# AOADMM-DataFusionFramework/Matlab-Code

Measured on AMD Instinct MI355X. Metric: AO-ADMM outer iters/sec (+ mode-1 MTTKRP GFLOP/s), 2000^3 rank-20 CP, higher is better.
Workload: dtype f32

## Files before the change

### matlab-code_amd/csrc/contract.hip

```cpp
#include "contract.h"
#include "device_utils.h"
#include "small_dev.h"

#include <algorithm>
#include <cstdlib>

namespace aoadmm {

typedef float f32x4 __attribute__((ext_vector_type(4)));
typedef double f64x2 __attribute__((ext_vector_type(2)));
typedef double f64x4 __attribute__((ext_vector_type(4)));

static constexpr int kTileRows = 128;
static constexpr int kGroup = 8;

struct KArgs {
  const void* X;
  const void* frag;
  void* T;
  int64_t tiles_per_batch, ntiles, batch_stride, M, ld, C, Cg, trows;
  int groups_per_chunk, R;
  int flush_every;
};

// ... 677 lines not shown
  const int64_t ng = g1 > g0 ? g1 - g0 : 0;
  const _Float16* xp = a.X + (blk * a.Cg + g0) * kGroupHalves + (m0 + r16) * kGroup16 + 8 * q;
  const f16x8* fp = reinterpret_cast<const f16x8*>(reinterpret_cast<const char*>(a.frag) + kFragHeader16) + g0 * (NT * 128) + lane;

  f32x4 acc[NT][8];
#pragma unroll
  for (int nt = 0; nt < NT; ++nt)
#pragma unroll
    for (int t = 0; t < 8; ++t) acc[nt][t] = f32x4{0.f, 0.f, 0.f, 0.f};

  f16x8 x0[8], x1[8], x2[8];
  f16x8 f0[NT][2], f1[NT][2], f2[NT][2];
#define AO_LOAD1(XS, GI, TL) XS[TL] = __builtin_nontemporal_load(reinterpret_cast<const f16x8*>(xp + (GI) * kGroupHalves + (TL) * (16 * kGroup16)));
#define AO_LOADF(FS, GI)                                                                             \
  {                                                                                                  \
    _Pragma("unroll") for (int nt = 0; nt < NT; ++nt) {                                              \
      FS[nt][0] = fp[(GI) * (NT * 128) + nt * 128];                                                  \
      FS[nt][1] = fp[(GI) * (NT * 128) + nt * 128 + 64];                                             \
    }                                                                                                \
  }
#define AO_LOAD_STAGE(XS, FS, GI)                                                                    \
  { _Pragma("unroll") for (int tl_ = 0; tl_ < 8; ++tl_) AO_LOAD1(XS, GI, tl_) AO_LOADF(FS, GI) }
#define AO_FMA_T(XS, FS, TL)                                                                         \
  {                                                                                                  \
    _Pragma("unroll") for (int nt = 0; nt < NT; ++nt) {                                              \
      acc[nt][TL] = __builtin_amdgcn_mfma_f32_16x16x32_f16(XS[TL], FS[nt][0], acc[nt][TL], 0, 0, 0); \
      acc[nt][TL] = __builtin_amdgcn_mfma_f32_16x16x32_f16(XS[TL], FS[nt][1], acc[nt][TL], 0, 0, 0); \
    }                                                                                                \
  }
#define AO_COMPUTE_STAGE(XS, FS) { _Pragma("unroll") for (int tl_ = 0; tl_ < 8; ++tl_) AO_FMA_T(XS, FS, tl_) }
#define AO_MIX_STAGE(XC, FC, XL, FL, GI)                                                             \
  {                                                                                                  \
    _Pragma("unroll") for (int tl_ = 0; tl_ < 8; ++tl_) {                                            \
      AO_FMA_T(XC, FC, tl_) AO_LOAD1(XL, GI, tl_)                                                    \
      if (tl_ == 7) AO_LOADF(FL, GI)                                                                 \
      __builtin_amdgcn_sched_barrier(0);                                                             \
    }                                                                                                \
  }
  if (ng > 0) AO_LOAD_STAGE(x0, f0, 0)
  if (ng > 1) AO_LOAD_STAGE(x1, f1, 1)
  int64_t g = 0;
  for (; g + 5 <= ng; g += 3) {
    AO_MIX_STAGE(x0, f0, x2, f2, g + 2)
    AO_MIX_STAGE(x1, f1, x0, f0, g + 3)
    AO_MIX_STAGE(x2, f2, x1, f1, g + 4)
  }
  for (; g + 3 <= ng; g += 3) {
    if (g + 2 < ng) AO_LOAD_STAGE(x2, f2, g + 2)
    AO_COMPUTE_STAGE(x0, f0)
    if (g + 3 < ng) AO_LOAD_STAGE(x0, f0, g + 3)
    AO_COMPUTE_STAGE(x1, f1)
    if (g + 4 < ng) AO_LOAD_STAGE(x1, f1, g + 4)
    AO_COMPUTE_STAGE(x2, f2)
  }
  if (g < ng) AO_COMPUTE_STAGE(x0, f0)
  if (g + 1 < ng) AO_COMPUTE_STAGE(x1, f1)
#undef AO_LOAD1
#undef AO_LOADF
#undef AO_LOAD_STAGE
#undef AO_FMA_T
#undef AO_COMPUTE_STAGE
#undef AO_MIX_STAGE
  extern __shared__ __attribute__((aligned(16))) float t_lds[];
  float* tl = t_lds + (threadIdx.x >> 6) * (kTileRows * a.R);
  const float* tinv = reinterpret_cast<const float*>(reinterpret_cast<const char*>(a.frag) + 512);
#pragma unroll
  for (int nt = 0; nt < NT; ++nt) {
    const int r = 16 * nt + r16;
    if (r < a.R) {
      const float ti = tinv[r];
#pragma unroll
      for (int t = 0; t < 8; ++t)
#pragma unroll
        for (int i = 0; i < 4; ++i) tl[(16 * t + 4 * q + i) * a.R + r] = acc[nt][t][i] * ti * a.inv_s;
    }
  }
  {
    const int n16 = kTileRows * a.R / 4;
    f32x4* dst = reinterpret_cast<f32x4*>(a.T + ((int64_t)chunk * a.trows + blk * 512 + m0) * a.R);
    const f32x4* src = reinterpret_cast<const f32x4*>(tl);
    for (int c = lane; c < n16; c += 64) __builtin_nontemporal_store(src[c], dst + c);
  }
}

static int nt_of(int R, int prec) {
  const int w = prec == AOADMM_PREC_F32 ? 32 : 16;
  return (R + w - 1) / w;
}
static int tile_rows(int prec) { return prec == AOADMM_PREC_F64 ? kTileRows64 : kTileRows; }

size_t ContractPlan::frag_bytes(int prec) const {
  if (prec == AOADMM_PREC_F16)
    return (size_t)kFragHeader16 + (size_t)cdiv(C, kGroup16) * nt_of(R, prec) * 2048;
  const int64_t Cg = cdiv(C, kGroup);
  return (size_t)(nt_of(R, prec) * 1024 + 1152) * Cg + 8192;
}

ContractPlan make_plan(int64_t nbatch, int64_t batch_stride, int64_t M, int64_t ld, int64_t C, int R,
                       int prec) {
  ContractPlan p;
  const bool half = prec == AOADMM_PREC_F16;
  p.tprec = half ? AOADMM_PREC_F32 : prec;
  p.nbatch = nbatch; p.batch_stride = batch_stride; p.M = M; p.ld = ld; p.C = C; p.R = R;
  const int gcols = half ? kGroup16 : kGroup;
  const int64_t Cg = cdiv(C, gcols);
  const int64_t ntiles = nbatch * cdiv(M, tile_rows(prec));
  int64_t nchunk = 1;
  if (prec != AOADMM_PREC_F64) nchunk = cdiv(Cg, 2048 / gcols);
  if (ntiles < 2048) {
    int64_t want = cdiv(2048, ntiles);
    const int64_t gmin = 128 / gcols;
    int64_t maxc = Cg / gmin > 0 ? Cg / gmin : 1;
    if (want > maxc) want = maxc;
    if (want > nchunk) nchunk = want;
  }
  if (nchunk > 65535) nchunk = 65535;
  p.nchunk = (int)nchunk;
  return p;
}

ContractPlan make_lead_plan(int64_t M, int64_t ld, int64_t C, int R) {
  ContractPlan p;
  p.tprec = AOADMM_PREC_F32;
  p.nbatch = 1; p.batch_stride = 0; p.M = M; p.ld = ld; p.C = C; p.R = R;
  p.lead = true;
  const int64_t nch = cdiv(C, kLeadKC);
  p.nchunk = (int)cdiv(nch, 2048 / kLeadKC);
  return p;
}

static void launch_contract_lead(const void* X, const ContractPlan& pl, const double* F, int64_t ldF, void* frag_ws,
                                 void* T, hipStream_t s, hipEvent_t ev0, hipEvent_t ev1) {
  const int64_t Cg = cdiv(pl.C, kGroup);
  AO_REQUIRE(pl.ld % 4 == 0 && pl.ld >= 4, "f32 layout must be padded to 4");
  LArgs a;
  a.X = (const float*)X; a.frag = (const float*)frag_ws; a.T = (float*)T;
  a.M = pl.M; a.ld = pl.ld; a.C = pl.C; a.Cg = Cg; a.R = pl.R;
  a.chunks_per_slice = (int)cdiv(cdiv(pl.C, kLeadKC), pl.nchunk);
  const int64_t nblk = cdiv(pl.M, kLeadRows);
  AO_REQUIRE(nblk < (int64_t)2147483647, "tensor too large for one launch");
  dim3 grid((unsigned)nblk, (unsigned)pl.nchunk);
  const size_t sh = (size_t)2 * kLeadRows * kLeadStride * sizeof(float);
  const int nt16 = (pl.R + 15) / 16;
  const int64_t Cg16 = cdiv(pl.C, 16) + 1;
  const int64_t total = (int64_t)nt16 * Cg16 * 256;
  pack_frag_lead16_f32<<<(unsigned)cdiv(total, 256), 256, 0, s>>>(F, ldF, pl.C, pl.R, nt16, Cg16, (float*)frag_ws);
  AO_KERNEL_CHECK();
#define AO_SET(K) ensure_dynamic_lds(reinterpret_cast<const void*>(K), (int)sh);
  if (nt16 == 1) AO_SET(contract_lead16_f32<1>)
  else if (nt16 == 2) AO_SET(contract_lead16_f32<2>)
  else if (nt16 == 3) AO_SET(contract_lead16_f32<3>)
  else if (nt16 == 4) AO_SET(contract_lead16_f32<4>)
#undef AO_SET
  if (ev0) AO_HIP(hipEventRecord(ev0, s));
  if (nt16 == 1) contract_lead16_f32<1><<<grid, 256, sh, s>>>(a);
  else if (nt16 == 2) contract_lead16_f32<2><<<grid, 256, sh, s>>>(a);
  else if (nt16 == 3) contract_lead16_f32<3><<<grid, 256, sh, s>>>(a);
  else if (nt16 == 4) contract_lead16_f32<4><<<grid, 256, sh, s>>>(a);
  else throw Error(AOADMM_ERR_UNSUPPORTED, "rank > 64 not supported");
  if (ev1) AO_HIP(hipEventRecord(ev1, s));
  AO_KERNEL_CHECK();
}

static void launch_contract_half(const void* X, const ContractPlan& pl, const double* F, int64_t ldF, void* frag_ws,
                                 void* T, hipStream_t s, hipEvent_t ev0, hipEvent_t ev1) {
  AO_REQUIRE(pl.on_copy && !pl.lead && pl.M == 512 && pl.ld == 512 && pl.tprec == AOADMM_PREC_F32,
             "internal: a half operand is streamed from its pass copies only");
  const int64_t Cg = cdiv(pl.C, kGroup16);
  AO_REQUIRE(pl.batch_stride == 512 * kGroup16 * Cg && pl.nbatch > 0 && pl.C > 0, "internal: half pass copy and plan disagree");
  const int NT = nt_of(pl.R, AOADMM_PREC_F16);
  char* ws = reinterpret_cast<char*>(frag_ws);
  double* tsc = reinterpret_cast<double*>(ws);
  float* tinv = reinterpret_cast<float*>(ws + 512);
  frag16_scales_k<<<(unsigned)pl.R, 256, 0, s>>>(F, ldF, pl.C, tsc, tinv);
  AO_KERNEL_CHECK();
  pack_frag16_f16<<<(unsigned)cdiv(Cg * NT * 128, 256), 256, 0, s>>>(F, ldF, pl.C, pl.R, NT, Cg, tsc,
                                                                    reinterpret_cast<f16x8*>(ws + kFragHeader16));
  AO_KERNEL_CHECK();
  KArgs16 a;
  a.X = reinterpret_cast<const _Float16*>(X); a.frag = frag_ws; a.T = reinterpret_cast<float*>(T);
  a.ntiles = pl.nbatch * 4; a.Cg = Cg; a.trows = pl.trows();
  a.groups_per_chunk = (int)cdiv(Cg, pl.nchunk);
  a.R = pl.R;
  a.inv_s = (float)(1.0 / pl.xscale);
  AO_REQUIRE(pl.nbatch < (int64_t)2147483647, "tensor too large for one launch");
  const dim3 grid((unsigned)pl.nbatch, (unsigned)pl.nchunk);
  const size_t tsh = (size_t)4 * kTileRows * pl.R * sizeof(float);
#define AO_GO(K) { if (tsh > 65536) ensure_dynamic_lds(reinterpret_cast<const void*>(K), (int)tsh); if (ev0) AO_HIP(hipEventRecord(ev0, s)); K<<<grid, 256, tsh, s>>>(a); }
  if (NT == 1) AO_GO(contract16_f16<1>)
  else if (NT == 2) AO_GO(contract16_f16<2>)
  else if (NT == 3) AO_GO(contract16_f16<3>)
  else if (NT == 4) AO_GO(contract16_f16<4>)
  else throw Error(AOADMM_ERR_UNSUPPORTED, "rank > 64 not supported");
#undef AO_GO
  if (ev1) AO_HIP(hipEventRecord(ev1, s));
  AO_KERNEL_CHECK();
}

void launch_contract(const void* X, int prec, const ContractPlan& pl, const double* F, int64_t ldF,
                     void* frag_ws, void* T, hipStream_t s, hipEvent_t ev0, hipEvent_t ev1) {
  AO_REQUIRE(pl.R >= 1 && pl.R <= kMaxRank, "rank %d outside [1,%d]", pl.R, kMaxRank);
  if (prec == AOADMM_PREC_F16) {
    launch_contract_half(X, pl, F, ldF, frag_ws, T, s, ev0, ev1);
    return;
  }
  AO_REQUIRE(prec == AOADMM_PREC_F32 || prec == AOADMM_PREC_F64, "bad precision id %d", prec);
  AO_REQUIRE(pl.tprec == prec, "contraction plan and tensor precision disagree");
  if (pl.lead) {
    AO_REQUIRE(prec == AOADMM_PREC_F32, "leading-mode contraction exists for fp32 tensors only");
    launch_contract_lead(X, pl, F, ldF, frag_ws, T, s, ev0, ev1);
    return;
  }
  const int64_t Cg = cdiv(pl.C, kGroup);
  KArgs a;
  a.X = X; a.frag = frag_ws; a.T = T;
  a.tiles_per_batch = cdiv(pl.M, tile_rows(prec));
  a.ntiles = pl.nbatch * a.tiles_per_batch;
  a.batch_stride = pl.batch_stride; a.M = pl.M; a.ld = pl.ld; a.C = pl.C; a.Cg = Cg;
  a.trows = pl.trows();
  a.groups_per_chunk = (int)cdiv(Cg, pl.nchunk);
  a.R = pl.R;
  AO_REQUIRE(a.ntiles > 0 && pl.C > 0, "empty contraction");
  dim3 grid((unsigned)cdiv(a.ntiles, 4), (unsigned)pl.nchunk);
  AO_REQUIRE(cdiv(a.ntiles, 4) < (int64_t)2147483647, "tensor too large for one launch");
  if (prec == AOADMM_PREC_F32) {
    AO_REQUIRE(pl.ld % 4 == 0 && pl.M % 4 == 0 && pl.batch_stride % 4 == 0, "f32 layout must be padded to 4");
    const int rem = pl.R % 16;
    const bool ex = pl.R > 16 && rem >= 1 && rem <= 4;
    const int nt16 = ex ? pl.R / 16 : (pl.R + 15) / 16;
    const int64_t total = (int64_t)nt16 * Cg * 128 + (ex ? Cg * 32 : 0);
    pack_frag16_f32<<<(unsigned)cdiv(total, 256), 256, 0, s>>>(F, ldF, pl.C, pl.R, nt16, ex ? 1 : 0, Cg, (float*)frag_ws);
    AO_KERNEL_CHECK();
    size_t tsh = (size_t)4 * kTileRows * pl.R * sizeof(float);
    a.flush_every = kFlushEvery;
    if (nt16 == 1) tsh = (size_t)4 * 16384;
#define AO_GO(K) { if (tsh > 65536) ensure_dynamic_lds(reinterpret_cast<const void*>(K), (int)tsh); if (ev0) AO_HIP(hipEventRecord(ev0, s)); K<<<grid, 256, tsh, s>>>(a); }
    if (nt16 == 1 && !ex) AO_GO((contract16_f32<1, false, true>))
    else if (nt16 == 1) AO_GO((contract16_f32<1, true, true>))
    else if (nt16 == 2 && !ex) AO_GO((contract16_f32<2, false>))
    else if (nt16 == 2) AO_GO((contract16_f32<2, true>))
    else if (nt16 == 3 && !ex) AO_GO((contract16_f32<3, false>))
    else if (nt16 == 3) AO_GO((contract16_f32<3, true>))
    else if (nt16 == 4) AO_GO((contract16_f32<4, false>))
    else throw Error(AOADMM_ERR_UNSUPPORTED, "rank > 64 not supported");
#undef AO_GO
  } else {
    AO_REQUIRE(pl.ld % 2 == 0 && pl.M % 2 == 0 && pl.batch_stride % 2 == 0, "f64 layout must be padded to 2");
    const int rem = pl.R % 16;
    const bool ex = pl.R > 16 && rem >= 1 && rem <= 4;
    const int nt16 = ex ? pl.R / 16 : (pl.R + 15) / 16;
    const int64_t total = (int64_t)nt16 * Cg * 128 + (ex ? Cg * 32 : 0);
    pack_frag_f64<<<(unsigned)cdiv(total, 256), 256, 0, s>>>(F, ldF, pl.C, pl.R, nt16, ex ? 1 : 0, Cg, (double*)frag_ws);
    AO_KERNEL_CHECK();
    const size_t tsh = (size_t)4 * kTileRows64 * pl.R * sizeof(double);
#define AO_GO(K) { if (tsh > 65536) ensure_dynamic_lds(reinterpret_cast<const void*>(K), (int)tsh); if (ev0) AO_HIP(hipEventRecord(ev0, s)); K<<<grid, 256, tsh, s>>>(a); }
    if (nt16 == 1 && !ex) AO_GO((contract_f64<1, false>))
    else if (nt16 == 1) AO_GO((contract_f64<1, true>))
    else if (nt16 == 2 && !ex) AO_GO((contract_f64<2, false>))
    else if (nt16 == 2) AO_GO((contract_f64<2, true>))
    else if (nt16 == 3 && !ex) AO_GO((contract_f64<3, false>))
    else if (nt16 == 3) AO_GO((contract_f64<3, true>))
    else if (nt16 == 4) AO_GO((contract_f64<4, false>))
    else throw Error(AOADMM_ERR_UNSUPPORTED, "rank > 64 not supported");
#undef AO_GO
  }
  if (ev1) AO_HIP(hipEventRecord(ev1, s));
  AO_KERNEL_CHECK();
}

__global__ void factor_rowmajor_k(const double* __restrict__ F, int64_t ldF, int64_t rows, int R,
                                  double* __restrict__ Ft) {
  const int64_t idx = (int64_t)blockIdx.x * blockDim.x + threadIdx.x;
  if (idx >= rows * R) return;
  const int r = (int)(idx / rows);
  const int64_t a = idx - (int64_t)r * rows;
  Ft[a * R + r] = F[a + ldF * r];
}
static void factor_rowmajor(const double* F, int64_t ldF, int64_t rows, int R, double* Ft, hipStream_t s) {
  factor_rowmajor_k<<<(unsigned)cdiv(rows * R, 256), 256, 0, s>>>(F, ldF, rows, R, Ft);
  AO_KERNEL_CHECK();
}

template <typename TT, int VEC> struct TVec;
template <> struct TVec<float, 4> { typedef float type __attribute__((ext_vector_type(4))); };
template <> struct TVec<float, 1> { typedef float type; };
template <> struct TVec<double, 2> { typedef double type __attribute__((ext_vector_type(2))); };
template <> struct TVec<double, 1> { typedef double type; };
template <typename TT, int VEC>
__device__ __forceinline__ void fma_vec(double (&acc)[VEC], const TT* __restrict__ tp, const double* __restrict__ fp) {
  typedef typename TVec<TT, VEC>::type V;
  const V tv = __builtin_nontemporal_load(reinterpret_cast<const V*>(tp));
  if constexpr (VEC == 1) {
    acc[0] += (double)tv * fp[0];
  } else {
#pragma unroll
    for (int v = 0; v < VEC; ++v) acc[v] += (double)tv[v] * fp[v];
  }
}

template <typename TT, int VEC>
struct RVec {
  typename TVec<TT, VEC>::type t;
  double f[VEC];
  __device__ __forceinline__ void load(const TT* __restrict__ tp, const double* __restrict__ fp) {
    t = __builtin_nontemporal_load(reinterpret_cast<const typename TVec<TT, VEC>::type*>(tp));
#pragma unroll
    for (int v = 0; v < VEC; ++v) f[v] = fp[v];
  }
  __device__ __forceinline__ void fma(double (&acc)[VEC]) const {
    if constexpr (VEC == 1) {
      acc[0] += (double)t * f[0];
    } else {
#pragma unroll
      for (int v = 0; v < VEC; ++v) acc[v] += (double)t[v] * f[v];
    }
  }
};

template <typename TT, int VEC>
__global__ void reduce_inner_k(const TT* __restrict__ T, int nchunk, int64_t trows, int64_t A, int64_t Apad, int R,
                               const double* __restrict__ FaT, double scale, double* __restrict__ out,
                               int64_t ldOut, int rowmajor, int has_sys, SysBuild sys) {
  extern __shared__ double sh[];
  if (has_sys && blockIdx.x == 0) { sys_build_rider(sys); return; }
  const int64_t b = (int64_t)blockIdx.x - has_sys;
  const int t = threadIdx.x;
  const int64_t n = A * R, step = (int64_t)blockDim.x * VEC;
  double s0[VEC], s1[VEC], s2[VEC], s3[VEC];
#pragma unroll
  for (int v = 0; v < VEC; ++v) { s0[v] = 0; s1[v] = 0; s2[v] = 0; s3[v] = 0; }
  for (int ch = 0; ch < nchunk; ++ch) {
    const TT* Tb = T + ((int64_t)ch * trows + Apad * b) * R;
    int64_t e = (int64_t)t * VEC;
    for (; e + 3 * step < n; e += 4 * step) {
      RVec<TT, VEC> q0, q1, q2, q3;
      q0.load(Tb + e, FaT + e);
      q1.load(Tb + e + step, FaT + e + step);
      q2.load(Tb + e + 2 * step, FaT + e + 2 * step);
      q3.load(Tb + e + 3 * step, FaT + e + 3 * step);
      __builtin_amdgcn_sched_barrier(0);
      q0.fma(s0); q1.fma(s1); q2.fma(s2); q3.fma(s3);
    }
    for (; e < n; e += step) fma_vec<TT, VEC>(s0, Tb + e, FaT + e);
  }
#pragma unroll
  for (int v = 0; v < VEC; ++v) sh[t * VEC + v] = (s0[v] + s1[v]) + (s2[v] + s3[v]);
  __syncthreads();
  if (t < R) {
    const int nA = blockDim.x * VEC / R;
    double tot = 0.0;
    for (int i = 0; i < nA; ++i) tot += sh[i * R + t];
    if (rowmajor) out[b * R + t] = scale * tot;
    else out[b + ldOut * t] = scale * tot;
  }
}

template <typename TT, int VEC>
__global__ void reduce_inner2_k(const TT* __restrict__ T, int nchunk, int64_t trows, int64_t A, int64_t Apad, int64_t B,
                                int R, const double* __restrict__ FaT, double scale, double* __restrict__ out,
                                int64_t ldOut, int rowmajor, int has_sys, SysBuild sys) {
  extern __shared__ double sh[];
  if (has_sys && blockIdx.x == 0) { sys_build_rider(sys); return; }
  const int64_t b0 = 2 * ((int64_t)blockIdx.x - has_sys);
  const bool two = b0 + 1 < B;
  const int64_t b1 = two ? b0 + 1 : b0;
  const int t = threadIdx.x;
  const int64_t n = A * R, step = (int64_t)blockDim.x * VEC;
  double a0[VEC], a1[VEC], c0[VEC], c1[VEC];
#pragma unroll
  for (int v = 0; v < VEC; ++v) { a0[v] = 0; a1[v] = 0; c0[v] = 0; c1[v] = 0; }
  for (int ch = 0; ch < nchunk; ++ch) {
    const TT* Ta = T + ((int64_t)ch * trows + Apad * b0) * R;
    const TT* Tc = T + ((int64_t)ch * trows + Apad * b1) * R;
    int64_t e = (int64_t)t * VEC;
    for (; e + step < n; e += 2 * step) {
      RVec<TT, VEC> q0, q1, p0, p1;
      q0.load(Ta + e, FaT + e);
      q1.load(Ta + e + step, FaT + e + step);
      p0.t = __builtin_nontemporal_load(reinterpret_cast<const typename TVec<TT, VEC>::type*>(Tc + e));
      p1.t = __builtin_nontemporal_load(reinterpret_cast<const typename TVec<TT, VEC>::type*>(Tc + e + step));
      __builtin_amdgcn_sched_barrier(0);
#pragma unroll
      for (int v = 0; v < VEC; ++v) { p0.f[v] = q0.f[v]; p1.f[v] = q1.f[v]; }
      q0.fma(a0); q1.fma(a1); p0.fma(c0); p1.fma(c1);
    }
    for (; e < n; e += step) {
      RVec<TT, VEC> q0, p0;
      q0.load(Ta + e, FaT + e);
      p0.t = __builtin_nontemporal_load(reinterpret_cast<const typename TVec<TT, VEC>::type*>(Tc + e));
#pragma unroll
      for (int v = 0; v < VEC; ++v) p0.f[v] = q0.f[v];
      q0.fma(a0); p0.fma(c0);
    }
  }
  const int nt = blockDim.x * VEC;
#pragma unroll
  for (int v = 0; v < VEC; ++v) { sh[t * VEC + v] = a0[v] + a1[v]; sh[nt + t * VEC + v] = c0[v] + c1[v]; }
  __syncthreads();
  if (t < 2 * R) {
    const int which = t / R, r = t % R;
    if (which == 0 || two) {
      const int nA = nt / R;
      double tot = 0.0;
      for (int i = 0; i < nA; ++i) tot += sh[which * nt + i * R + r];
      const int64_t b = which ? b1 : b0;
      if (rowmajor) out[b * R + r] = scale * tot;
      else out[b + ldOut * r] = scale * tot;
    }
  }
}

size_t reduce_factor_scratch_bytes(int64_t rows, int R) { return (size_t)rows * R * sizeof(double); }

template <typename TT, int VEC>
static void launch_inner_t(const void* T, int nchunk, int64_t trows, int64_t A, int64_t Apad, int64_t B, int R,
                           const double* FaT, double scale, double* out, int64_t ldOut, hipStream_t s, int rowmajor,
                           const SysBuild* sys) {
  const int hs = sys ? 1 : 0;
  const SysBuild sb = sys ? *sys : SysBuild();
  const int rq = R / VEC;
  int threads = 256 / rq * rq;
  if (threads < rq) threads = rq;
  if (threads * VEC < R) threads = (R + VEC - 1) / VEC;
  if (B >= 1024 && 2 * R <= threads) {
    reduce_inner2_k<TT, VEC><<<(unsigned)((B + 1) / 2 + hs), threads, (size_t)2 * threads * VEC * sizeof(double), s>>>(
        (const TT*)T, nchunk, trows, A, Apad, B, R, FaT, scale, out, ldOut, rowmajor, hs, sb);
    return;
  }
  reduce_inner_k<TT, VEC><<<(unsigned)(B + hs), threads, (size_t)threads * VEC * sizeof(double), s>>>(
      (const TT*)T, nchunk, trows, A, Apad, R, FaT, scale, out, ldOut, rowmajor, hs, sb);
}

static bool sys_can_ride(const SysBuild* sys, int threads_min = 64) {
  return sys != nullptr && sys->R >= 1 && sys->R <= kSysRiderMaxR && threads_min >= 64;
}

bool launch_reduce_inner(const void* T, int tprec, int nchunk, int64_t trows, int64_t A, int64_t Apad,
                         int64_t B, int R, const double* Fa, int64_t ldFa, double scale,
                         double* out, int64_t ldOut, double* ft_scratch, hipStream_t s, const double* FaT,
                         int rowmajor_out, const SysBuild* sys) {
  AO_REQUIRE((int64_t)B < 2147483647ll, "reduce_inner: too many output rows for one launch");
  {
    const int vec = tprec == AOADMM_PREC_F32 ? (R % 4 == 0 ? 4 : 1) : (R % 2 == 0 ? 2 : 1);
    const int rq = R / vec;
    int threads = 256 / rq * rq;
    if (threads < rq) threads = rq;
    if (threads * vec < R) threads = (R + vec - 1) / vec;
    if (!sys_can_ride(sys, threads)) sys = nullptr;
  }
  if (FaT) ft_scratch = const_cast<double*>(FaT);
  else factor_rowmajor(Fa, ldFa, A, R, ft_scratch, s);
  if (tprec == AOADMM_PREC_F32) {
    if (R % 4 == 0) launch_inner_t<float, 4>(T, nchunk, trows, A, Apad, B, R, ft_scratch, scale, out, ldOut, s, rowmajor_out, sys);
    else launch_inner_t<float, 1>(T, nchunk, trows, A, Apad, B, R, ft_scratch, scale, out, ldOut, s, rowmajor_out, sys);
  } else {
    if (R % 2 == 0) launch_inner_t<double, 2>(T, nchunk, trows, A, Apad, B, R, ft_scratch, scale, out, ldOut, s, rowmajor_out, sys);
    else launch_inner_t<double, 1>(T, nchunk, trows, A, Apad, B, R, ft_scratch, scale, out, ldOut, s, rowmajor_out, sys);
  }
  AO_KERNEL_CHECK();
  return sys != nullptr;
}

static void outer_geometry(int64_t A, int64_t B, int R, int vec, int& TA, int64_t& nblkA, int& SB) {
  const int rq = (R + vec - 1) / vec;
  TA = 256 / rq;
  if (TA < 1) TA = 1;
  nblkA = cdiv(A, TA);
  int64_t sb = cdiv(2048, nblkA);
  if (sb > 64) sb = 64;
  if (sb > B) sb = B;
  if (sb < 1) sb = 1;
  SB = (int)sb;
}
static int outer_vec(int tprec, int R) {
  if (tprec == AOADMM_PREC_F32) return R % 4 == 0 ? 4 : 1;
  return R % 2 == 0 ? 2 : 1;
}

size_t reduce_outer_scratch_bytes(int64_t A, int64_t B, int R) {
  size_t worst = 0;
  for (int vec : {1, 2, 4}) {
    int TA, SB; int64_t nb;
    outer_geometry(A, B, R, vec, TA, nb, SB);
    worst = std::max(worst, (size_t)SB * A * R * sizeof(double));
  }
  return worst;
}

template <typename TT, int VEC>
__global__ void reduce_outer_k(const TT* __restrict__ T, int nchunk, int64_t trows, int64_t A,
                               int64_t Apad, int64_t B, int R, int TA, const double* __restrict__ FbT,
                               double* __restrict__ part, int has_sys, SysBuild sys) {
  if (has_sys && blockIdx.x == 0) {
    if (blockIdx.y == 0) sys_build_rider(sys);
    return;
  }
  const int t = threadIdx.x;
  const int rq = R / VEC;
  const int al = t / rq, r = (t - al * rq) * VEC;
  const int64_t a = ((int64_t)blockIdx.x - has_sys) * TA + al;
  const int SB = gridDim.y, sb = blockIdx.y;
  const int64_t bper = (B + SB - 1) / SB;
  const int64_t b0 = sb * bper;
  int64_t b1 = b0 + bper;
  if (b1 > B) b1 = B;
  if (al >= TA || a >= A) return;
  const int64_t bs = Apad * R;
  double s0[VEC], s1[VEC], s2[VEC], s3[VEC];
#pragma unroll
  for (int v = 0; v < VEC; ++v) { s0[v] = 0; s1[v] = 0; s2[v] = 0; s3[v] = 0; }
  for (int ch = 0; ch < nchunk; ++ch) {
    const TT* Tc = T + (int64_t)ch * trows * R + a * R + r;
    const double* Fr = FbT + r;
    int64_t b = b0;
    for (; b + 3 < b1; b += 4) {
      RVec<TT, VEC> q0, q1, q2, q3;
      q0.load(Tc + bs * b, Fr + b * R);
      q1.load(Tc + bs * (b + 1), Fr + (b + 1) * R);
      q2.load(Tc + bs * (b + 2), Fr + (b + 2) * R);
      q3.load(Tc + bs * (b + 3), Fr + (b + 3) * R);
      __builtin_amdgcn_sched_barrier(0);
      q0.fma(s0); q1.fma(s1); q2.fma(s2); q3.fma(s3);
    }
    for (; b < b1; ++b) fma_vec<TT, VEC>(s0, Tc + bs * b, Fr + b * R);
  }
#pragma unroll
  for (int v = 0; v < VEC; ++v) part[((int64_t)sb * A + a) * R + r + v] = (s0[v] + s1[v]) + (s2[v] + s3[v]);
}

__global__ void reduce_outer_fin(const double* __restrict__ part, int SB, int64_t A, int R, double scale,
                                 double* __restrict__ out, int64_t ldOut, int rowmajor) {
  int64_t idx = (int64_t)blockIdx.x * blockDim.x + threadIdx.x;
  if (idx >= A * R) return;
  const int64_t a = idx / R;
  const int r = (int)(idx - a * R);
  double t0 = 0.0, t1 = 0.0;
  int s = 0;
  const int64_t ar = A * R;
  for (; s + 7 < SB; s += 8) {
    const double v0 = part[(int64_t)s * ar + idx], v1 = part[(int64_t)(s + 1) * ar + idx];
    const double v2 = part[(int64_t)(s + 2) * ar + idx], v3 = part[(int64_t)(s + 3) * ar + idx];
    const double v4 = part[(int64_t)(s + 4) * ar + idx], v5 = part[(int64_t)(s + 5) * ar + idx];
    const double v6 = part[(int64_t)(s + 6) * ar + idx], v7 = part[(int64_t)(s + 7) * ar + idx];
    t0 += v0; t1 += v1; t0 += v2; t1 += v3; t0 += v4; t1 += v5; t0 += v6; t1 += v7;
  }
  for (; s + 1 < SB; s += 2) {
    t0 += part[(int64_t)s * ar + idx];
    t1 += part[(int64_t)(s + 1) * ar + idx];
  }
  if (s < SB) t0 += part[(int64_t)s * ar + idx];
  if (rowmajor) out[idx] = scale * (t0 + t1);
  else out[a + ldOut * r] = scale * (t0 + t1);
}

template <typename TT, int VEC>
static void launch_outer_t(const void* T, int nchunk, int64_t trows, int64_t A, int64_t Apad, int64_t B, int R,
                           const double* FbT, double* scratch, int& SB, hipStream_t s, const SysBuild* sys) {
  int TA; int64_t nb;
  outer_geometry(A, B, R, VEC, TA, nb, SB);
  int threads = TA * (R / VEC);
  threads = (threads + 63) / 64 * 64;
  const int hs = sys ? 1 : 0;
  reduce_outer_k<TT, VEC><<<dim3((unsigned)(nb + hs), (unsigned)SB), threads, 0, s>>>((const TT*)T, nchunk, trows, A, Apad, B,
                                                                                    R, TA, FbT, scratch, hs, sys ? *sys : SysBuild());
}

bool launch_reduce_outer(const void* T, int tprec, int nchunk, int64_t trows, int64_t A, int64_t Apad,
                         int64_t B, int R, const double* Fb, int64_t ldFb, double scale,
                         double* out, int64_t ldOut, double* scratch, double* ft_scratch, hipStream_t s,
                         const double* FbT, int rowmajor_out, const SysBuild* sys) {
  if (!sys_can_ride(sys)) sys = nullptr;
  if (FbT) ft_scratch = const_cast<double*>(FbT);
  else factor_rowmajor(Fb, ldFb, B, R, ft_scratch, s);
  int SB = 1;
  const int vec = outer_vec(tprec, R);
  if (tprec == AOADMM_PREC_F32) {
    if (vec == 4) launch_outer_t<float, 4>(T, nchunk, trows, A, Apad, B, R, ft_scratch, scratch, SB, s, sys);
    else launch_outer_t<float, 1>(T, nchunk, trows, A, Apad, B, R, ft_scratch, scratch, SB, s, sys);
  } else {
    if (vec == 2) launch_outer_t<double, 2>(T, nchunk, trows, A, Apad, B, R, ft_scratch, scratch, SB, s, sys);
    else launch_outer_t<double, 1>(T, nchunk, trows, A, Apad, B, R, ft_scratch, scratch, SB, s, sys);
  }
  AO_KERNEL_CHECK();
  reduce_outer_fin<<<(unsigned)cdiv(A * R, 256), 256, 0, s>>>(scratch, SB, A, R, scale, out, ldOut, rowmajor_out);
  AO_KERNEL_CHECK();
  return sys != nullptr;
}

template <typename TT, int RMAX>
__global__ __launch_bounds__(256) void small_mttkrp_k(SmallMttkrp a, int has_sys, SysBuild sys) {
  extern __shared__ double sf[];
  if (has_sys && blockIdx.x == 0) { sys_build_rider(sys); return; }
  const int row = (int)blockIdx.x - has_sys;
  const int R = a.R, Na = a.Na, Nb = a.Nb;
  double* fa = sf;
  double* fb = sf + (size_t)Na * R;
  double* red = fb + (size_t)(Nb > 0 ? Nb : 1) * R;
  for (int e = threadIdx.x; e < Na * R; e += 256) { const int i = e / R, r = e - i * R; fa[e] = a.Fa[i + a.lda * r]; }
  for (int e = threadIdx.x; e < Nb * R; e += 256) { const int i = e / R, r = e - i * R; fb[e] = a.Fb ? a.Fb[i + a.ldb * r] : 1.0; }
  __syncthreads();
  const TT* X = reinterpret_cast<const TT*>(a.X) + (int64_t)row * a.sn;
  double acc[RMAX];
#pragma unroll
  for (int r = 0; r < RMAX; ++r) acc[r] = 0.0;
  const int npairs = Na * Nb;
  for (int p = threadIdx.x; p < npairs; p += 256) {
    const int ia = p % Na, ib = p / Na;
    const double x = (double)X[(int64_t)ia * a.sa + (int64_t)ib * a.sb];
#pragma unroll
    for (int r = 0; r < RMAX; ++r)
      if (r < R) acc[r] += x * (fa[ia * R + r] * fb[ib * R + r]);
  }
  const int lane = threadIdx.x & 63, w = threadIdx.x >> 6;
#pragma unroll
  for (int r = 0; r < RMAX; ++r) {
    const double v = wave_sum(acc[r]);
    if (lane == 0) red[w * RMAX + r] = v;
  }
  __syncthreads();
  if ((int)threadIdx.x < R) {
    const int r = threadIdx.x;
    const double tot = (red[r] + red[RMAX + r]) + (red[2 * RMAX + r] + red[3 * RMAX + r]);
    a.out[row + a.ldOut * r] = a.scale * tot;
  }
}

bool small_mttkrp_ok(int64_t elems, int nd, const int64_t* dims, int R) {
  const bool off = getenv("AOADMM_NO_SMALL_MTTKRP") != nullptr;
  if (off || elems > kSmallMttkrpElems || !(nd == 2 || nd == 3) || R > 16) return false;
  int64_t sum = 0;
  for (int i = 0; i < nd; ++i) sum += dims[i];
  return (size_t)(sum * R + 64) * sizeof(double) <= 40 * 1024;
}

bool small_mttkrp(const SmallMttkrp& a, int prec, int64_t rows, hipStream_t s, const SysBuild* sys) {
  if (!sys_can_ride(sys)) sys = nullptr;
  const int hs = sys ? 1 : 0;
  const SysBuild sb = sys ? *sys : SysBuild();
  AO_REQUIRE(a.R >= 1 && a.R <= 16 && rows >= 1 && a.Na >= 1 && a.Nb >= 1, "small_mttkrp: bad sizes");
  const int rmax = a.R <= 4 ? 4 : (a.R <= 8 ? 8 : 16);
  const size_t lds = ((size_t)(a.Na + a.Nb) * a.R + 4 * rmax) * sizeof(double);
  AO_REQUIRE(lds <= 48 * 1024, "small_mttkrp: factors do not fit LDS");
#define AO_SM(TT, RM) small_mttkrp_k<TT, RM><<<(unsigned)(rows + hs), 256, lds, s>>>(a, hs, sb)
  if (prec == AOADMM_PREC_F32) { if (rmax == 4) AO_SM(float, 4); else if (rmax == 8) AO_SM(float, 8); else AO_SM(float, 16); }
  else { if (rmax == 4) AO_SM(double, 4); else if (rmax == 8) AO_SM(double, 8); else AO_SM(double, 16); }
#undef AO_SM
  AO_KERNEL_CHECK();
  return sys != nullptr;
}

template <typename TT>
__global__ void t_to_colmajor_k(const TT* __restrict__ T, int nchunk, int64_t trows, int64_t A, int R,
                                double scale, double* __restrict__ out, int64_t ldOut) {
  int64_t idx = (int64_t)blockIdx.x * blockDim.x + threadIdx.x;
  if (idx >= A * R) return;
  const int64_t a = idx / R;
  const int r = (int)(idx - a * R);
  double tot = 0.0;
  for (int ch = 0; ch < nchunk; ++ch) tot += (double)T[(int64_t)ch * trows * R + idx];
  out[a + ldOut * r] = scale * tot;
}

void launch_t_to_colmajor(const void* T, int tprec, int nchunk, int64_t trows, int64_t A, int R, double scale,
                          double* out, int64_t ldOut, hipStream_t s) {
  const unsigned nb = (unsigned)cdiv(A * R, 256);
  if (tprec == AOADMM_PREC_F32) t_to_colmajor_k<float><<<nb, 256, 0, s>>>((const float*)T, nchunk, trows, A, R, scale, out, ldOut);
  else t_to_colmajor_k<double><<<nb, 256, 0, s>>>((const double*)T, nchunk, trows, A, R, scale, out, ldOut);
  AO_KERNEL_CHECK();
}

}
```

Baseline: 128.9.

## Generalize inner reduction to multi-slice blocks and restructure outer reduction with LDS staging

The inner reduction kernel now handles 2 or 4 output slices per block with a deeper unroll, so each loaded factor value is reused across more T slices. The outer reduction becomes a persistent grid-stride kernel that stages factor tiles in LDS, double-buffers T loads in batches of eight, and adjusts the TA tile so row strides align to 128 bytes. The aim is less redundant factor traffic from global memory and better latency hiding on this bandwidth-bound contraction. In exchange it adds register pressure, block-wide barriers and LDS use, which may lower occupancy.

```diff
diff --git a/matlab-code_amd/csrc/contract.hip b/matlab-code_amd/csrc/contract.hip
--- a/matlab-code_amd/csrc/contract.hip
+++ b/matlab-code_amd/csrc/contract.hip
@@ -1003,11 +1003,14 @@
 struct RVec {
   typename TVec<TT, VEC>::type t;
   double f[VEC];
-  __device__ __forceinline__ void load(const TT* __restrict__ tp, const double* __restrict__ fp) {
+  __device__ __forceinline__ void load_t(const TT* __restrict__ tp) {
     t = __builtin_nontemporal_load(reinterpret_cast<const typename TVec<TT, VEC>::type*>(tp));
+  }
+  __device__ __forceinline__ void load_f(const double* __restrict__ fp) {
 #pragma unroll
     for (int v = 0; v < VEC; ++v) f[v] = fp[v];
   }
+  __device__ __forceinline__ void load(const TT* __restrict__ tp, const double* __restrict__ fp) { load_t(tp); load_f(fp); }
   __device__ __forceinline__ void fma(double (&acc)[VEC]) const {
     if constexpr (VEC == 1) {
       acc[0] += (double)t * f[0];
@@ -1056,55 +1059,70 @@
   }
 }
 
-template <typename TT, int VEC>
-__global__ void reduce_inner2_k(const TT* __restrict__ T, int nchunk, int64_t trows, int64_t A, int64_t Apad, int64_t B,
+template <typename TT, int VEC, int NS, int U>
+__global__ __launch_bounds__(256, NS == 4 ? 2 : 4) void reduce_innerN_k(const TT* __restrict__ T, int nchunk, int64_t trows, int64_t A, int64_t Apad, int64_t B,
                                 int R, const double* __restrict__ FaT, double scale, double* __restrict__ out,
                                 int64_t ldOut, int rowmajor, int has_sys, SysBuild sys) {
+  typedef typename TVec<TT, VEC>::type V;
   extern __shared__ double sh[];
   if (has_sys && blockIdx.x == 0) { sys_build_rider(sys); return; }
-  const int64_t b0 = 2 * ((int64_t)blockIdx.x - has_sys);
-  const bool two = b0 + 1 < B;
-  const int64_t b1 = two ? b0 + 1 : b0;
+  const int64_t b0 = NS * ((int64_t)blockIdx.x - has_sys);
   const int t = threadIdx.x;
   const int64_t n = A * R, step = (int64_t)blockDim.x * VEC;
-  double a0[VEC], a1[VEC], c0[VEC], c1[VEC];
-#pragma unroll
-  for (int v = 0; v < VEC; ++v) { a0[v] = 0; a1[v] = 0; c0[v] = 0; c1[v] = 0; }
+  double a0[NS][VEC], a1[NS][VEC];
+#pragma unroll
+  for (int i = 0; i < NS; ++i)
+#pragma unroll
+    for (int v = 0; v < VEC; ++v) { a0[i][v] = 0; a1[i][v] = 0; }
   for (int ch = 0; ch < nchunk; ++ch) {
-    const TT* Ta = T + ((int64_t)ch * trows + Apad * b0) * R;
-    const TT* Tc = T + ((int64_t)ch * trows + Apad * b1) * R;
+    const TT* Tp[NS];
+#pragma unroll
+    for (int i = 0; i < NS; ++i) Tp[i] = T + ((int64_t)ch * trows + Apad * (b0 + i < B ? b0 + i : B - 1)) * R;
     int64_t e = (int64_t)t * VEC;
-    for (; e + step < n; e += 2 * step) {
-      RVec<TT, VEC> q0, q1, p0, p1;
-      q0.load(Ta + e, FaT + e);
-      q1.load(Ta + e + step, FaT + e + step);
-      p0.t = __builtin_nontemporal_load(reinterpret_cast<const typename TVec<TT, VEC>::type*>(Tc + e));
-      p1.t = __builtin_nontemporal_load(reinterpret_cast<const typename TVec<TT, VEC>::type*>(Tc + e + step));
+    for (; e + (U - 1) * step < n; e += U * step) {
+      RVec<TT, VEC> q[U][NS];
+#pragma unroll
+      for (int u = 0; u < U; ++u) {
+        q[u][0].load(Tp[0] + e + u * step, FaT + e + u * step);
+#pragma unroll
+        for (int i = 1; i < NS; ++i) q[u][i].t = __builtin_nontemporal_load(reinterpret_cast<const V*>(Tp[i] + e + u * step));
+      }
       __builtin_amdgcn_sched_barrier(0);
 #pragma unroll
-      for (int v = 0; v < VEC; ++v) { p0.f[v] = q0.f[v]; p1.f[v] = q1.f[v]; }
-      q0.fma(a0); q1.fma(a1); p0.fma(c0); p1.fma(c1);
-    }
-    for (; e < n; e += step) {
-      RVec<TT, VEC> q0, p0;
-      q0.load(Ta + e, FaT + e);
-      p0.t = __builtin_nontemporal_load(reinterpret_cast<const typename TVec<TT, VEC>::type*>(Tc + e));
-#pragma unroll
-      for (int v = 0; v < VEC; ++v) p0.f[v] = q0.f[v];
-      q0.fma(a0); p0.fma(c0);
+      for (int u = 0; u < U; ++u)
+#pragma unroll
+        for (int i = 0; i < NS; ++i) {
+#pragma unroll
+          for (int v = 0; v < VEC; ++v) q[u][i].f[v] = q[u][0].f[v];
+          if (u % 2 == 0) q[u][i].fma(a0[i]); else q[u][i].fma(a1[i]);
+        }
+    }
+    for (int u = 0; e < n; e += step, ++u) {
+      RVec<TT, VEC> q[NS];
+      q[0].load(Tp[0] + e, FaT + e);
+#pragma unroll
+      for (int i = 1; i < NS; ++i) q[i].t = __builtin_nontemporal_load(reinterpret_cast<const V*>(Tp[i] + e));
+#pragma unroll
+      for (int i = 0; i < NS; ++i) {
+#pragma unroll
+        for (int v = 0; v < VEC; ++v) q[i].f[v] = q[0].f[v];
+        if (u % 2 == 0) q[i].fma(a0[i]); else q[i].fma(a1[i]);
+      }
     }
   }
   const int nt = blockDim.x * VEC;
 #pragma unroll
-  for (int v = 0; v < VEC; ++v) { sh[t * VEC + v] = a0[v] + a1[v]; sh[nt + t * VEC + v] = c0[v] + c1[v]; }
+  for (int i = 0; i < NS; ++i)
+#pragma unroll
+    for (int v = 0; v < VEC; ++v) sh[i * nt + t * VEC + v] = a0[i][v] + a1[i][v];
   __syncthreads();
-  if (t < 2 * R) {
+  if (t < NS * R) {
     const int which = t / R, r = t % R;
-    if (which == 0 || two) {
+    const int64_t b = b0 + which;
+    if (b < B) {
       const int nA = nt / R;
       double tot = 0.0;
       for (int i = 0; i < nA; ++i) tot += sh[which * nt + i * R + r];
-      const int64_t b = which ? b1 : b0;
       if (rowmajor) out[b * R + r] = scale * tot;
       else out[b + ldOut * r] = scale * tot;
     }
@@ -1124,8 +1142,13 @@
   if (threads < rq) threads = rq;
   if (threads * VEC < R) threads = (R + VEC - 1) / VEC;
   if (B >= 1024 && 2 * R <= threads) {
-    reduce_inner2_k<TT, VEC><<<(unsigned)((B + 1) / 2 + hs), threads, (size_t)2 * threads * VEC * sizeof(double), s>>>(
-        (const TT*)T, nchunk, trows, A, Apad, B, R, FaT, scale, out, ldOut, rowmajor, hs, sb);
+    const size_t lds = (size_t)threads * VEC * sizeof(double);
+    if (4 * R <= threads)
+      reduce_innerN_k<TT, VEC, 4, 4><<<(unsigned)(cdiv(B, 4) + hs), threads, 4 * lds, s>>>(
+          (const TT*)T, nchunk, trows, A, Apad, B, R, FaT, scale, out, ldOut, rowmajor, hs, sb);
+    else
+      reduce_innerN_k<TT, VEC, 2, 4><<<(unsigned)(cdiv(B, 2) + hs), threads, 2 * lds, s>>>(
+          (const TT*)T, nchunk, trows, A, Apad, B, R, FaT, scale, out, ldOut, rowmajor, hs, sb);
     return;
   }
   reduce_inner_k<TT, VEC><<<(unsigned)(B + hs), threads, (size_t)threads * VEC * sizeof(double), s>>>(
@@ -1188,45 +1211,114 @@
   return worst;
 }
 
+static int outer_lds_rows(int R) { return std::max(8, (int)(16384 / ((size_t)R * sizeof(double))) / 8 * 8); }
+
 template <typename TT, int VEC>
-__global__ void reduce_outer_k(const TT* __restrict__ T, int nchunk, int64_t trows, int64_t A,
-                               int64_t Apad, int64_t B, int R, int TA, const double* __restrict__ FbT,
-                               double* __restrict__ part, int has_sys, SysBuild sys) {
-  if (has_sys && blockIdx.x == 0) {
-    if (blockIdx.y == 0) sys_build_rider(sys);
-    return;
-  }
+__device__ __forceinline__ void outer_load8(RVec<TT, VEC> (&q)[8], const TT* __restrict__ Tc, int64_t bs, int64_t b, int64_t be) {
+#pragma unroll
+  for (int u = 0; u < 8; ++u) q[u].load_t(Tc + bs * (b + u < be ? b + u : be - 1));
+}
+template <typename TT, int VEC>
+__device__ __forceinline__ void outer_fma_full(RVec<TT, VEC> (&q)[8], const double* Fr, int R, double (&s0)[VEC],
+                                               double (&s1)[VEC], double (&s2)[VEC], double (&s3)[VEC]) {
+#pragma unroll
+  for (int u = 0; u < 4; ++u) q[u].load_f(Fr + u * R);
+  q[0].fma(s0); q[1].fma(s1); q[2].fma(s2); q[3].fma(s3);
+  __builtin_amdgcn_sched_barrier(0);
+#pragma unroll
+  for (int u = 4; u < 8; ++u) q[u].load_f(Fr + u * R);
+  q[4].fma(s0); q[5].fma(s1); q[6].fma(s2); q[7].fma(s3);
+}
+template <typename TT, int VEC>
+__device__ __forceinline__ void outer_fma_tail(RVec<TT, VEC> (&q)[8], const double* Fr, int R, int64_t n, double (&s0)[VEC],
+                                               double (&s1)[VEC], double (&s2)[VEC], double (&s3)[VEC]) {
+  if (n >= 4) {
+#pragma unroll
+    for (int u = 0; u < 4; ++u) q[u].load_f(Fr + u * R);
+    q[0].fma(s0); q[1].fma(s1); q[2].fma(s2); q[3].fma(s3);
+#pragma unroll
+    for (int u = 4; u < 7; ++u)
+      if (u < n) { q[u].load_f(Fr + u * R); q[u].fma(s0); }
+  } else {
+#pragma unroll
+    for (int u = 0; u < 3; ++u)
+      if (u < n) { q[u].load_f(Fr + u * R); q[u].fma(s0); }
+  }
+}
+
+template <typename TT, int VEC>
+__global__ __launch_bounds__(256, 2) void reduce_outer_k(const TT* __restrict__ T, int nchunk, int64_t trows, int64_t A,
+                                                      int64_t Apad, int64_t B, int R, int TA, int64_t nblkA, int SB, int KT,
+                                                      const double* __restrict__ FbT, double* __restrict__ part,
+                                                      int has_sys, SysBuild sys) {
+  extern __shared__ double fs[];
+  if (has_sys && blockIdx.x == 0) { sys_build_rider(sys); return; }
   const int t = threadIdx.x;
   const int rq = R / VEC;
   const int al = t / rq, r = (t - al * rq) * VEC;
-  const int64_t a = ((int64_t)blockIdx.x - has_sys) * TA + al;
-  const int SB = gridDim.y, sb = blockIdx.y;
   const int64_t bper = (B + SB - 1) / SB;
-  const int64_t b0 = sb * bper;
-  int64_t b1 = b0 + bper;
-  if (b1 > B) b1 = B;
-  if (al >= TA || a >= A) return;
   const int64_t bs = Apad * R;
-  double s0[VEC], s1[VEC], s2[VEC], s3[VEC];
-#pragma unroll
-  for (int v = 0; v < VEC; ++v) { s0[v] = 0; s1[v] = 0; s2[v] = 0; s3[v] = 0; }
-  for (int ch = 0; ch < nchunk; ++ch) {
-    const TT* Tc = T + (int64_t)ch * trows * R + a * R + r;
-    const double* Fr = FbT + r;
-    int64_t b = b0;
-    for (; b + 3 < b1; b += 4) {
-      RVec<TT, VEC> q0, q1, q2, q3;
-      q0.load(Tc + bs * b, Fr + b * R);
-      q1.load(Tc + bs * (b + 1), Fr + (b + 1) * R);
-      q2.load(Tc + bs * (b + 2), Fr + (b + 2) * R);
-      q3.load(Tc + bs * (b + 3), Fr + (b + 3) * R);
-      __builtin_amdgcn_sched_barrier(0);
-      q0.fma(s0); q1.fma(s1); q2.fma(s2); q3.fma(s3);
-    }
-    for (; b < b1; ++b) fma_vec<TT, VEC>(s0, Tc + bs * b, Fr + b * R);
-  }
-#pragma unroll
-  for (int v = 0; v < VEC; ++v) part[((int64_t)sb * A + a) * R + r + v] = (s0[v] + s1[v]) + (s2[v] + s3[v]);
+  const int64_t nitems = nblkA * SB, G = (int64_t)gridDim.x - has_sys;
+  for (int64_t item = (int64_t)blockIdx.x - has_sys; item < nitems; item += G) {
+    const int64_t sb = item / nblkA;
+    const int64_t a = (item - sb * nblkA) * TA + al;
+    const int64_t b0 = sb * bper;
+    int64_t b1 = b0 + bper;
+    if (b1 > B) b1 = B;
+    const bool live = al < TA && a < A;
+    double s0[VEC], s1[VEC], s2[VEC], s3[VEC];
+#pragma unroll
+    for (int v = 0; v < VEC; ++v) { s0[v] = 0; s1[v] = 0; s2[v] = 0; s3[v] = 0; }
+    for (int ch = 0; ch < nchunk; ++ch) {
+      const TT* Tc = T + (int64_t)ch * trows * R + a * R + r;
+      for (int64_t bt = b0; bt < b1; bt += KT) {
+        const int64_t be = bt + KT < b1 ? bt + KT : b1;
+        RVec<TT, VEC> qa[8], qb[8];
+        if (live) outer_load8<TT, VEC>(qa, Tc, bs, bt, be);
+        if (ch == 0 || b1 - b0 > KT) {
+          __syncthreads();
+          const int64_t nf = (be - bt) * R;
+          const double* __restrict__ Fs = FbT + bt * R;
+          for (int64_t i0 = t; i0 < nf; i0 += 8 * (int64_t)blockDim.x) {
+            double fv[8];
+#pragma unroll
+            for (int k = 0; k < 8; ++k) { const int64_t i = i0 + k * (int64_t)blockDim.x; fv[k] = Fs[i < nf ? i : nf - 1]; }
+#pragma unroll
+            for (int k = 0; k < 8; ++k) { const int64_t i = i0 + k * (int64_t)blockDim.x; if (i < nf) fs[i] = fv[k]; }
+          }
+          __syncthreads();
+        }
+        if (!live) continue;
+        const double* Fr = fs + r;
+        const int64_t nfull = (be - bt) / 8, rem = (be - bt) - 8 * nfull;
+        const int64_t nbatch = nfull + (rem ? 1 : 0);
+        int64_t k = 0;
+        for (;;) {
+          if (k + 1 >= nbatch) break;
+          outer_load8<TT, VEC>(qb, Tc, bs, bt + 8 * (k + 1), be);
+          __builtin_amdgcn_sched_barrier(0);
+          outer_fma_full<TT, VEC>(qa, Fr + 8 * k * R, R, s0, s1, s2, s3);
+          ++k;
+          if (k + 1 >= nbatch) break;
+          outer_load8<TT, VEC>(qa, Tc, bs, bt + 8 * (k + 1), be);
+          __builtin_amdgcn_sched_barrier(0);
+          outer_fma_full<TT, VEC>(qb, Fr + 8 * k * R, R, s0, s1, s2, s3);
+          ++k;
+        }
+        if (k & 1) {
+          if (rem) outer_fma_tail<TT, VEC>(qb, Fr + 8 * k * R, R, rem, s0, s1, s2, s3);
+          else outer_fma_full<TT, VEC>(qb, Fr + 8 * k * R, R, s0, s1, s2, s3);
+        } else {
+          if (rem) outer_fma_tail<TT, VEC>(qa, Fr + 8 * k * R, R, rem, s0, s1, s2, s3);
+          else outer_fma_full<TT, VEC>(qa, Fr + 8 * k * R, R, s0, s1, s2, s3);
+        }
+      }
+    }
+    if (live) {
+#pragma unroll
+      for (int v = 0; v < VEC; ++v) part[((int64_t)sb * A + a) * R + r + v] = (s0[v] + s1[v]) + (s2[v] + s3[v]);
+    }
+  }
 }
 
 __global__ void reduce_outer_fin(const double* __restrict__ part, int SB, int64_t A, int R, double scale,
@@ -1254,16 +1346,29 @@
   else out[a + ldOut * r] = scale * (t0 + t1);
 }
 
+static constexpr int64_t kOuterResident = 256 * 2;
+
 template <typename TT, int VEC>
 static void launch_outer_t(const void* T, int nchunk, int64_t trows, int64_t A, int64_t Apad, int64_t B, int R,
                            const double* FbT, double* scratch, int& SB, hipStream_t s, const SysBuild* sys) {
   int TA; int64_t nb;
   outer_geometry(A, B, R, VEC, TA, nb, SB);
+  {
+    int ta = TA;
+    while (ta > 1 && ((size_t)ta * R * sizeof(TT)) % 128 != 0) --ta;
+    if (((size_t)ta * R * sizeof(TT)) % 128 == 0 && ((size_t)Apad * R * sizeof(TT)) % 128 == 0) { TA = ta; nb = cdiv(A, TA); }
+  }
   int threads = TA * (R / VEC);
   threads = (threads + 63) / 64 * 64;
   const int hs = sys ? 1 : 0;
-  reduce_outer_k<TT, VEC><<<dim3((unsigned)(nb + hs), (unsigned)SB), threads, 0, s>>>((const TT*)T, nchunk, trows, A, Apad, B,
-                                                                                    R, TA, FbT, scratch, hs, sys ? *sys : SysBuild());
+  const int64_t nitems = nb * SB;
+  int64_t rounds = cdiv(nitems, kOuterResident);
+  const int64_t grid = cdiv(nitems, rounds);
+  const int KT = outer_lds_rows(R);
+  const int64_t bper = cdiv(B, SB);
+  const size_t lds = (size_t)std::min<int64_t>(bper, KT) * R * sizeof(double);
+  reduce_outer_k<TT, VEC><<<(unsigned)(grid + hs), threads, lds, s>>>((const TT*)T, nchunk, trows, A, Apad, B, R, TA, nb, SB, KT,
+                                                                     FbT, scratch, hs, sys ? *sys : SysBuild());
 }
 
 bool launch_reduce_outer(const void* T, int tprec, int nchunk, int64_t trows, int64_t A, int64_t Apad,
```

New measurement: 129.1, median of 5. No clear change (+0.1%).
